# nabeelre/BTSbot

Measured on AMD Instinct MI355X. Metric: alerts/sec (63×63×3 triplet + 25 meta) train+infer, 1/2/4/8 MI355X, higher is better.
Workload: dtype bf16; 1 GPU; BASELINE.json configs[1]: ConvNeXt-pico multi-modal (mm_ConvNeXt) bf16 inference, batch=1024 synthetic triplets per GPU, inputs resident in HBM, logits+scores out; per_gpu_batch=1024, global_batch=1024, precision=bf16, weights=seeded random, layer-scale ~1, parallelism=1 independent replicas, batch-sharded, no collective, pipeline_depth=3

## Files before the change

btsbot_amd/csrc/device_math.h:

```cpp
#pragma once

struct h2x8 { f16x8 hi, lo; };
struct h2x4 { f16x4v hi, lo; };
__device__ __forceinline__ void split_f16(float v, _Float16& hi, _Float16& lo) {
  hi = (_Float16)v;
  lo = (_Float16)(v - (float)hi);
}
__device__ __forceinline__ h2x8 split8(const float (&v)[8]) {
  h2x8 o;
#pragma unroll
  for (int j = 0; j < 8; ++j) {
    _Float16 a, b;
    split_f16(v[j], a, b);
    o.hi[j] = a;
    o.lo[j] = b;
  }
  return o;
}
constexpr int AMAX_SUB = 16, AMAX_STRIDE = 32, AMAX_WORDS = AMAX_SUB * AMAX_STRIDE;
__device__ __forceinline__ int split_exp(const unsigned* amax) {
  if (amax == nullptr) return 0;
  unsigned m = 0;
#pragma unroll
  for (int i = 0; i < AMAX_SUB; ++i) m = max(m, amax[i * AMAX_STRIDE]);
// ... 38 lines not shown
template <> __device__ __forceinline__ float gelu_q<5>(float a) {
  float t = fmaf(a, -0.0004726569791655389f, 0.007079169600613161f);
  t = fmaf(a, t, -0.05181158088529847f);
  t = fmaf(a, t, -0.46001256950698816f);
  t = fmaf(a, t, -1.1507770495088248f);
  return fmaf(a, t, -1.000039487932206f);
}
__device__ __forceinline__ float relu_f(float x) {
  const int b = __float_as_int(x);
  return __int_as_float(b > 0 ? b : 0);
}
template <int DEG> __device__ __forceinline__ float gelu_poly(float x) {
  const float a = __builtin_fabsf(x);
  const float e = __builtin_amdgcn_exp2f(gelu_q<DEG>(a));
  return fmaf(-a, e, relu_f(x));
}
__device__ __forceinline__ void gelu_pk4(const float (&x)[8], f16x2v (&g)[4]) {
  const f16x2v c3 = {(_Float16)-0.024772998623334343f, (_Float16)-0.024772998623334343f};
  const f16x2v c2 = {(_Float16)-0.49926576060257244f, (_Float16)-0.49926576060257244f};
  const f16x2v c1 = {(_Float16)-1.1287482669759885f, (_Float16)-1.1287482669759885f};
  const f16x2v c0 = {(_Float16)-1.0036805164077327f, (_Float16)-1.0036805164077327f};
  const f16x2v z = {(_Float16)0.f, (_Float16)0.f};
  f16x2v xh[4], a[4], t[4];
  unsigned e[4];
#pragma unroll
  for (int i = 0; i < 4; ++i) xh[i] = __builtin_bit_cast(f16x2v, __builtin_amdgcn_cvt_pkrtz(x[2 * i], x[2 * i + 1]));
  __builtin_amdgcn_sched_barrier(0);
#pragma unroll
  for (int i = 0; i < 4; ++i) a[i] = __builtin_bit_cast(f16x2v, __builtin_bit_cast(unsigned, xh[i]) & 0x7fff7fffu);
  __builtin_amdgcn_sched_barrier(0);
#pragma unroll
  for (int i = 0; i < 4; ++i) t[i] = __builtin_elementwise_fma(a[i], c3, c2);
  __builtin_amdgcn_sched_barrier(0);
#pragma unroll
  for (int i = 0; i < 4; ++i) t[i] = __builtin_elementwise_fma(a[i], t[i], c1);
  __builtin_amdgcn_sched_barrier(0);
#pragma unroll
  for (int i = 0; i < 4; ++i) t[i] = __builtin_elementwise_fma(a[i], t[i], c0);
  __builtin_amdgcn_sched_barrier(0);
#pragma unroll
  for (int i = 0; i < 4; ++i) xh[i] = __builtin_elementwise_max(xh[i], z);
  __builtin_amdgcn_sched_barrier(0);
#pragma unroll
  for (int i = 0; i < 4; ++i) asm volatile("v_exp_f16_e32 %0, %1" : "=&v"(e[i]) : "v"(__builtin_bit_cast(unsigned, t[i])));
#pragma unroll
  for (int i = 0; i < 4; ++i)
    asm volatile("v_exp_f16_sdwa %0, %1 dst_sel:WORD_1 dst_unused:UNUSED_PRESERVE src0_sel:WORD_1"
                 : "+v"(e[i]) : "v"(__builtin_bit_cast(unsigned, t[i])));
  asm volatile("s_nop 0");
  __builtin_amdgcn_sched_barrier(0);
#pragma unroll
  for (int i = 0; i < 4; ++i) g[i] = __builtin_elementwise_fma(-a[i], __builtin_bit_cast(f16x2v, e[i]), xh[i]);
}
template <int DEG> __device__ __forceinline__ float gelu_dq(float a);
template <> __device__ __forceinline__ float gelu_dq<3>(float a) {
  float t = fmaf(a, 3.0f * -0.024772998623334343f, 2.0f * -0.49926576060257244f);
  return fmaf(a, t, -1.1287482669759885f);
}
template <> __device__ __forceinline__ float gelu_dq<5>(float a) {
  float t = fmaf(a, 5.0f * -0.0004726569791655389f, 4.0f * 0.007079169600613161f);
  t = fmaf(a, t, 3.0f * -0.05181158088529847f);
  t = fmaf(a, t, 2.0f * -0.46001256950698816f);
  return fmaf(a, t, -1.1507770495088248f);
}
template <int DEG> __device__ __forceinline__ float gelu_poly_grad(float x) {
  const float a = __builtin_fabsf(x);
  const float e = __builtin_amdgcn_exp2f(gelu_q<DEG>(a));
  const float d = e * fmaf(a * 0.6931471805599453f, gelu_dq<DEG>(a), 1.0f);
  return x > 0.0f ? 1.0f - d : d;
}
template <typename T> struct GeluDeg { static constexpr int value = 5; };
template <> struct GeluDeg<bf16_t> { static constexpr int value = 3; };
template <typename T> __device__ __forceinline__ float gelu_for(float x) { return gelu_poly<GeluDeg<T>::value>(x); }
template <> __device__ __forceinline__ float gelu_for<float>(float x) { return gelu_erf(x); }

__device__ __forceinline__ float gelu_grad(float x) {
  const float cdf = 0.5f * (1.0f + erff(x * 0.70710678118654752440f));
  const float pdf = 0.39894228040143267794f * __expf(-0.5f * x * x);
  return cdf + x * pdf;
}

__device__ __forceinline__ float silu_f(float x) { return x / (1.0f + __expf(-x)); }
__device__ __forceinline__ float silu_fast(float x) {
  return x * __builtin_amdgcn_rcpf(1.0f + __builtin_amdgcn_exp2f(-1.4426950408889634f * x));
}
template <typename T> __device__ __forceinline__ float silu_for(float x) { return silu_fast(x); }
template <> __device__ __forceinline__ float silu_for<float>(float x) { return silu_f(x); }

template <typename T> __device__ __forceinline__ float gelu_grad_for(float x) {
  return gelu_poly_grad<GeluDeg<T>::value>(x);
}
template <> __device__ __forceinline__ float gelu_grad_for<float>(float x) { return gelu_grad(x); }

template <typename T> __device__ __forceinline__ float to_f32(T x) { return (float)x; }

__device__ __forceinline__ float group16_sum(float v) {
#define BTS_DPP_ADD(ctrl)                                                                      \
  v += __builtin_bit_cast(float, __builtin_amdgcn_update_dpp(0, __builtin_bit_cast(int, v), ctrl, \
                                                             0xF, 0xF, true))
  BTS_DPP_ADD(0xB1);
  BTS_DPP_ADD(0x4E);
  BTS_DPP_ADD(0x141);
  BTS_DPP_ADD(0x140);
#undef BTS_DPP_ADD
  return v;
}
// ... 37 lines not shown
```

btsbot_amd/csrc/pack.hip:

```cpp
#include "ctx.h"
#include "head16.h"
#include "maxvit.h"
#include "stage3.h"

namespace {

template <typename T>
__global__ void cast_kernel(const float* __restrict__ s, T* __restrict__ d, int64_t n) {
  for (int64_t i = (int64_t)blockIdx.x * blockDim.x + threadIdx.x; i < n;
       i += (int64_t)gridDim.x * blockDim.x)
    d[i] = (T)s[i];
}

template <typename T>
__global__ void cast4_kernel(const float4* __restrict__ s, T* __restrict__ d, int64_t n4) {
  typedef __attribute__((ext_vector_type(4))) T t4;
  for (int64_t i = (int64_t)blockIdx.x * blockDim.x + threadIdx.x; i < n4;
       i += (int64_t)gridDim.x * blockDim.x) {
    const float4 v = s[i];
    *reinterpret_cast<t4*>(d + 4 * i) = t4{(T)v.x, (T)v.y, (T)v.z, (T)v.w};
  }
}

__global__ void transpose_kernel(const float* __restrict__ s, float* __restrict__ d, int R, int Cc) {
// ... 414 lines not shown
              [=](hipStream_t st) {
                return launch_pack_s2p(h->prec_down3(), h->mirror + d->w, nullptr, IMG(h, d->p_wp), ch, 4 * cin, 1, cin, nullptr, st);
              };
        job("down.p_w", &d->p_w, n * esz, FT, early && i == 1, PACK_DOWN, d->w, -1, ch, cin);
        job("down.p_wt", &d->p_wt, n * esz, if_tp, false, PACK_DOWN_T, d->w, -1, ch, cin);
        if (i == 3 && sc.stage2p)
          own("down.p_wp", &d->p_wp, 0, F, false, nullptr, [=](hipStream_t st) {
            return launch_pack_s2p(h->prec_down3(), h->mirror + d->w, nullptr, IMG(h, d->p_wp), ch, 4 * cin, 1, cin, nullptr, st);
          });
        if (i == 2 && sc.stage1)
          own("down.p_wp", &d->p_wp, n * esz, sc.s1_keep ? FT : F, false, nullptr, [=](hipStream_t st) {
            return launch_pack_frag32(h->prec_s01(), h->mirror + d->w, IMG(h, d->p_wp), ch, cin, st);
          });
        if (i == 1 && x2_s0) {
          own("down.p_x2_w", &d->p_x2_w, n * 2, F, false, nullptr, [=](hipStream_t st) {
            return launch_pack_down_split(h->mirror + d->w, IMG(h, d->p_x2_w), IMG(h, d->p_x2_wlo), ch, cin, st);
          });
          own("down.p_x2_wlo", &d->p_x2_wlo, n * 2, F, false, nullptr, nullptr);
        }
      }
      for (BlockPk& blk : h->blocks[i]) {
        BlockPk* b = &blk;
        const bool b_early = early && i == 0;
        job("p_dw", &b->p_dw, (size_t)49 * ch * 4, FT, b_early, PACK_TRANSPOSE_F32, b->dw_w, -1, ch, 49);
        job("p_fc1", &b->p_fc1, wb * esz, FT, b_early, PACK_CAST, b->fc1_w, -1, 4 * ch * ch, 1);
        job("p_fc2", &b->p_fc2, wb * esz, FT, false, PACK_CAST, b->fc2_w, -1, 4 * ch * ch, 1);
        const bool frag = (i == 2 && sc.stage2p) || (i == 3 && sc.stage3);
        if (i == 2 && sc.stage2p) {
          const unsigned t = sc.s2_keep ? IN_TRAIN : 0;
          job("p_w1p", &b->p_w1p, wb * esz, t, false, PACK_FRAG, b->fc1_w, -1, 4 * ch, ch).launch = [=](hipStream_t st) {
            return launch_pack_s2p(h->prec_tail(), h->mirror + b->fc1_w, nullptr, IMG(h, b->p_w1p), 4 * ch, ch, 0, 0,
                                   reinterpret_cast<float*>(IMG(h, b->p_scales)), st);
          };
          job("p_w2p", &b->p_w2p, wb * esz, t, false, PACK_FRAG, b->fc2_w, b->gamma, ch, 4 * ch).launch = [=](hipStream_t st) {
            return launch_pack_s2p(h->prec_tail(), h->mirror + b->fc2_w, h->mirror + b->gamma, IMG(h, b->p_w2p), ch, 4 * ch, 0, 0,
                                   reinterpret_cast<float*>(IMG(h, b->p_scales)) + 2, st);
          };
        }
        job("p_fc1t", &b->p_fc1t, wb * esz, if_tp, false, PACK_TRANSPOSE_CAST, b->fc1_w, -1, 4 * ch, ch);
        job("p_fc2t", &b->p_fc2t, wb * esz, if_tp, false, PACK_TRANSPOSE_CAST, b->fc2_w, b->gamma, ch, 4 * ch);
        if (!h->x2 && s2mlp_bwd_supported(prec, ch)) {
          const unsigned t = tp && sc.s2mlp ? FT : 0;
          ImageEntry& e1 = job("p_w1tp", &b->p_w1tp, wb * 2, t, false, PACK_TFRAG, b->fc1_w, -1, 4 * ch, ch);
          e1.reads = &b->p_fc1t;
          e1.launch = [=](hipStream_t st) { return launch_pack_frag16(IMG(h, b->p_fc1t), IMG(h, b->p_w1tp), ch, 4 * ch, st); };
          ImageEntry& e2 = job("p_w2tp", &b->p_w2tp, wb * 2, t, false, PACK_TFRAG, b->fc2_w, b->gamma, ch, 4 * ch);
          e2.reads = &b->p_fc2t;
          e2.launch = [=](hipStream_t st) { return launch_pack_frag16(IMG(h, b->p_fc2t), IMG(h, b->p_w2tp), 4 * ch, ch, st); };
        }
        own("p_fc2g", &b->p_fc2g, wb * esz, F | ((i == 0 && sc.s0_keep) || (i == 1 && sc.s1_keep) ? IN_TRAIN : 0), b_early, nullptr,
            [=](hipStream_t st) {
              return launch_rowscale_cast(h->cfg.precision, h->mirror + b->fc2_w, h->mirror + b->gamma, IMG(h, b->p_fc2g), ch, 4 * ch, st);
            });
        if (i == 0 && sc.stage0 && h->prec_s01() == BTSBOT_BF16)
          own("p_fc2g_h", &b->p_fc2g_h, wb * 2, F, false, nullptr, [=](hipStream_t st) {
            return launch_rowscale_cast(BTSBOT_F16, h->mirror + b->fc2_w, h->mirror + b->gamma, IMG(h, b->p_fc2g_h), ch, 4 * ch, st);
          });
        if (frag) {
          const bool s3 = i == 3;
          own("p_scales", &b->p_scales, 64, 0, false, nullptr, nullptr);
          own("p_w1p", &b->p_w1p, s3 ? wb * esz : 0, F, false, nullptr, [=](hipStream_t st) {
            float* sc = reinterpret_cast<float*>(IMG(h, b->p_scales));
            const float* w = h->mirror + b->fc1_w;
            return s3 ? launch_pack_s3(h->prec_tail(), w, nullptr, IMG(h, b->p_w1p), 4 * ch, ch, 1, sc, st)
                      : launch_pack_s2p(h->prec_tail(), w, nullptr, IMG(h, b->p_w1p), 4 * ch, ch, 0, 0, sc, st);
          });
          own("p_w2p", &b->p_w2p, s3 ? wb * esz : 0, F, false, nullptr, [=](hipStream_t st) {
            float* sc = reinterpret_cast<float*>(IMG(h, b->p_scales)) + 2;
            const float *w = h->mirror + b->fc2_w, *g = h->mirror + b->gamma;
            return s3 ? launch_pack_s3(h->prec_tail(), w, g, IMG(h, b->p_w2p), ch, 4 * ch, 0, sc, st)
                      : launch_pack_s2p(h->prec_tail(), w, g, IMG(h, b->p_w2p), ch, 4 * ch, 0, 0, sc, st);
          });
        }
        if (i == 1 && sc.stage1)
          own("p_s0par", &b->p_s0par, s1par_bytes(), F, false, &b->p_dw, [=](hipStream_t st) {
            const float* m = h->mirror;
            return launch_pack_s1par(h->prec_s01(), IMG_F32(h, b->p_dw), m + b->dw_b, m + b->ln_w, m + b->ln_b, IMG(h, b->p_s0par), st);
          });
        if (i == 0 && sc.stage0)
          own("p_s0par", &b->p_s0par, s0par_bytes(), F, false, &b->p_dw, [=](hipStream_t st) {
            const float* m = h->mirror;
            return launch_pack_s0par(h->prec_s01(), IMG_F32(h, b->p_dw), m + b->dw_b, m + b->ln_w, m + b->ln_b, m + b->fc1_b,
                                     m + b->fc2_b, m + b->gamma, IMG(h, b->p_s0par), st);
          });
        if (i == 1 && sc.s1_keep)
          own("p_s0par_t", &b->p_s0par_t, s1par_bytes(), if_tp, false, &b->p_dw, [=](hipStream_t st) {
            const float* m = h->mirror;
            return launch_pack_s1par(BTSBOT_F16, IMG_F32(h, b->p_dw), m + b->dw_b, m + b->ln_w, m + b->ln_b, IMG(h, b->p_s0par_t), st);
          });
        if (i == 0 && sc.s0_keep)
          own("p_s0par_t", &b->p_s0par_t, s0par_bytes(), if_tp, b_early, &b->p_dw, [=](hipStream_t st) {
            const float* m = h->mirror;
            return launch_pack_s0par(BTSBOT_F16, IMG_F32(h, b->p_dw), m + b->dw_b, m + b->ln_w, m + b->ln_b, m + b->fc1_b,
                                     m + b->fc2_b, m + b->gamma, IMG(h, b->p_s0par_t), st);
          });
        if (h->x2 && ((i == 0 && sc.stage0) || (i == 1 && sc.stage1))) {
          own("p_x2_w1", &b->p_x2_w1, wb * 2, F, false, nullptr, [=](hipStream_t st) {
            return launch_cast(BTSBOT_F16, h->mirror + b->fc1_w, IMG(h, b->p_x2_w1), (int64_t)4 * ch * ch, st);
          });
          own("p_x2_w2g", &b->p_x2_w2g, wb * 2, F, false, nullptr, [=](hipStream_t st) {
            return launch_rowscale_cast(BTSBOT_F16, h->mirror + b->fc2_w, h->mirror + b->gamma, IMG(h, b->p_x2_w2g), ch, 4 * ch, st);
          });
          own("p_x2_w1lo", &b->p_x2_w1lo, wb * 2, F, false, nullptr, [=](hipStream_t st) {
            return launch_rowscale_cast_lo(h->mirror + b->fc1_w, nullptr, IMG(h, b->p_x2_w1lo), 4 * ch, ch, st);
          });
          own("p_x2_w2glo", &b->p_x2_w2glo, wb * 2, F, false, nullptr, [=](hipStream_t st) {
            return launch_rowscale_cast_lo(h->mirror + b->fc2_w, h->mirror + b->gamma, IMG(h, b->p_x2_w2glo), ch, 4 * ch, st);
// ... 229 lines not shown
```

btsbot_amd/csrc/stage1b.hip:

```cpp
#include "stage0.h"
#include "stage_regs.h"
#include <type_traits>

namespace {

constexpr int C = 128, HW = 7, PA = 49, G = 2, NPX = G * PA, CT = 4, HID = 512, KS1 = 8;
constexpr int CN = 256, PO = 9;
constexpr int PITCH = 2 * C + 16;
static_assert(C == StageRegs<CT>::C && PITCH == StageRegs<CT>::PITCH, "ln_regs / regs_to_map derive both from CT");
constexpr int MAPB = NPX * PITCH;
constexpr int CHUNKB = 16384, HALFB = CHUNKB / 2, NCH = HID / 32, NSLOT = 3;
constexpr int PL_ROW = 136 * 8, PL_XQ = 8 * PL_ROW, PL_AL = 2 * PL_XQ, PLB = G * PL_AL;
constexpr int OFF_PL = 2 * CHUNKB;
constexpr int LNP = 4 * C + 16;
template <bool X2> struct S1L {
  static constexpr int PLANES = X2 ? 2 : 1;
  static constexpr int SLB = X2 ? 2 * HALFB : HALFB;
  static constexpr int OFF_W2X = OFF_PL + PLANES * PLB;
  static constexpr int OFF_B1 = OFF_W2X + (X2 ? 2 * SLB : 0);
  static constexpr int OFF_LNW = OFF_B1 + (HID + C) * 4;
  static constexpr int LDS_BYTES = OFF_LNW + 2 * C * 4;
  static_assert(4 * SLB <= PLANES * PLB, "W1 slots + W2 slot 0 inside the planar images");
  static_assert(NPX * LNP <= OFF_PL + PLB && NPX * LNP <= OFF_B1, "the fp32 image lies in ring slots 0, 1 + the planar image");
};
static_assert(MAPB <= 2 * CHUNKB && S1L<false>::LDS_BYTES <= 75264 && S1L<true>::LDS_BYTES <= 160 * 1024, "LDS layout");
constexpr int TW_R = 21, TW_BYTES = TW_R * C * 4 * 4 * 2;
constexpr int PARB = TW_BYTES + 3 * C * 4;
constexpr int PARB_X2 = 2 * TW_BYTES + 3 * C * 4;

#define SC_STAMP(i)                                                                \
  do {                                                                             \
    if (a.stamps != nullptr && blockIdx.x == 0 && threadIdx.x == 0) a.stamps[i] = clock64(); \
    if (a.wgt != nullptr && threadIdx.x == 0 && ((i) == 0 || (i) == 13))           \
      a.wgt[2 * blockIdx.x + ((i) == 13)] = wall_clock64();                        \
  } while (0)

template <typename T, int LOPLANE = 0, bool SAT = false>
__device__ __forceinline__ void regs_to_planar(const f32x16 (&x)[CT], unsigned char* pl, int p, int h) {
  const int al = p >= PA ? 1 : 0, pp = p - al * PA;
  const int y = pp / HW, xx = pp - y * HW;
  unsigned char* dst = pl + al * PL_AL + (xx >> 2) * PL_XQ + y * PL_ROW + (xx & 3) * 2 + h * 32;
#pragma unroll
  for (int ct = 0; ct < CT; ++ct)
#pragma unroll
    for (int r = 0; r < 16; ++r) {
      const T hi = (T)(SAT ? __builtin_amdgcn_fmed3f(x[ct][r], -65504.0f, 65504.0f) : x[ct][r]);
      *reinterpret_cast<T*>(dst + (ct * 32 + 8 * (r >> 2) + (r & 3)) * 8) = hi;
      if (LOPLANE > 0) *reinterpret_cast<T*>(dst + LOPLANE + (ct * 32 + 8 * (r >> 2) + (r & 3)) * 8) = (T)(x[ct][r] - (float)hi);
    }
}

template <typename T, bool X2, int WPS = 2, bool KEEP = false>
__global__ __launch_bounds__(256, WPS) void stage1b_kernel(Stage1Args a) {
  using frag = typename Mfma<T>::frag;
  using DT = typename std::conditional<KEEP, f16_t, T>::type;
  using frag4 = typename Mfma<DT>::frag4;
  extern __shared__ __attribute__((aligned(16))) unsigned char smem[];
  unsigned char* pl = smem + OFF_PL;
  unsigned char* stg = smem;
  using L = S1L<X2>;
  constexpr int SLB = L::SLB;
  constexpr int PLO = X2 ? PLB : 0;
  float* b1s = reinterpret_cast<float*>(smem + L::OFF_B1);
  float* b2s = b1s + HID;
  float* lnws = reinterpret_cast<float*>(smem + L::OFF_LNW);
  float* lnbs = lnws + C;
  auto w1slot = [&](int sl) { return pl + sl * SLB; };
  auto w2slot = [&](int sl) { return sl == 0 ? pl + 3 * SLB : (X2 ? smem + L::OFF_W2X : smem) + (sl - 1) * SLB; };

  const int tid = threadIdx.x, lane = tid & 63, wave = __builtin_amdgcn_readfirstlane(tid >> 6);
  const int lr = lane & 31, h = lane >> 5;
  const bool w1wave = wave < 2;
  const int a0 = blockIdx.x * G;
  const int nal = min(G, a.B - a0);
  const int p = wave * 32 + lr;
  const bool live = p < nal * PA;
  const bool inmap = p < NPX;
  const int pm = inmap ? p : 0;
  const int lnrow = pm * LNP + h * 32;
  SC_STAMP(0);
  auto zero_pads = [&]() {
#pragma unroll
    for (int pn = 0; pn < L::PLANES; ++pn) {
      unsigned char* pb = pl + pn * PLB;
      for (int i = tid; i < 4 * PL_ROW / 16; i += 256) {
        const int blk = i / (PL_ROW / 16), o = i - blk * (PL_ROW / 16);
        *reinterpret_cast<uint4*>(pb + (blk >> 1) * PL_AL + (blk & 1) * PL_XQ + 7 * PL_ROW + o * 16) = make_uint4(0u, 0u, 0u, 0u);
      }
      for (int i = tid; i < G * HW * C; i += 256) {
        const int al = i / (HW * C), r = (i / C) % HW, c = i % C;
        *reinterpret_cast<unsigned short*>(pb + al * PL_AL + PL_XQ + r * PL_ROW + c * 8 + 6) = 0;
      }
    }
  };
  zero_pads();
  const float* xsrc = a.x_in + ((size_t)a0 * PA + (live ? p : 0)) * C;
  float* xscr = a.scratch + ((size_t)a0 * PA + (live ? p : 0)) * C;
  auto load_x = [&](const float* src, f32x16 (&x)[CT]) {
#pragma unroll
    for (int ct = 0; ct < CT; ++ct)
#pragma unroll
      for (int qd = 0; qd < 4; ++qd) {
        const float4 v4 = *reinterpret_cast<const float4*>(src + ct * 32 + 8 * qd + 4 * h);
        x[ct][4 * qd + 0] = live ? v4.x : 0.f;
        x[ct][4 * qd + 1] = live ? v4.y : 0.f;
        x[ct][4 * qd + 2] = live ? v4.z : 0.f;
        x[ct][4 * qd + 3] = live ? v4.w : 0.f;
// ... 287 lines not shown
#define LS(i) do { __builtin_amdgcn_sched_barrier(0); if (ch == 6 || ch == 7) lts[i + 8 * (ch - 6)] = __builtin_amdgcn_s_memtime(); __builtin_amdgcn_sched_barrier(0); } while (0)
#else
#define LS(i)
#endif
      f32x16 hacc[2];
      frag a1[KS1];
      {
        wait_vm<(X2 ? 8 : 4) + 16>();
        asm volatile("s_waitcnt lgkmcnt(0)" ::: "memory");
        __builtin_amdgcn_s_barrier();
        bias_acc(0, hacc[0]);
        read_a1(0, a1);
#pragma unroll
        for (int ks = 0; ks < KS1; ++ks) {
          if (X2) {
            hacc[0] = Mfma<T>::m32(a1l[ks], xf[ks], hacc[0]);
            hacc[0] = Mfma<T>::m32(a1[ks], xfl[ks], hacc[0]);
          }
          hacc[0] = Mfma<T>::m32(a1[ks], xf[ks], hacc[0]);
        }
        __builtin_amdgcn_sched_barrier(0);
        wait_vm<0>();
        asm volatile("s_waitcnt lgkmcnt(0)" ::: "memory");
        __builtin_amdgcn_s_barrier();
        bias_acc(1, hacc[1]);
        read_a1(1, a1);
        __builtin_amdgcn_sched_barrier(0);
#pragma unroll
        for (int ct = 0; ct < CT; ++ct)
#pragma unroll
          for (int qd = 0; qd < 4; ++qd) {
            const f32x4 bv = lds4(b2s + ct * 32 + 8 * qd + 4 * h);
            const float4 v4 = xt[4 * ct + qd];
            x[ct][4 * qd + 0] = (live ? v4.x : 0.f) + bv[0];
            x[ct][4 * qd + 1] = (live ? v4.y : 0.f) + bv[1];
            x[ct][4 * qd + 2] = (live ? v4.z : 0.f) + bv[2];
            x[ct][4 * qd + 3] = (live ? v4.w : 0.f) + bv[3];
          }
#pragma unroll
        for (int ct = 0; ct < CT; ++ct) asm volatile("" : "+v"(x[ct]));
        __builtin_amdgcn_sched_barrier(0);
        if (w1wave) issue(3);
      }
      auto step = [&](auto last_c, int ch, f32x16& hc, f32x16& hn) {
        constexpr bool LAST = decltype(last_c)::value;
        LS(0);
        wait_vm<X2 ? 8 : 4>();
        LS(1);
        asm volatile("s_waitcnt lgkmcnt(0)" ::: "memory");
#ifndef S1_EXP_NOBAR
        __builtin_amdgcn_s_barrier();
#endif
        LS(2);
        frag a2[CT][2], a2l[X2 ? CT : 1][2];
        const unsigned char* w2s = w2slot(ch % NSLOT);
#pragma unroll
        for (int ct = 0; ct < CT; ++ct)
#pragma unroll
          for (int s2 = 0; s2 < 2; ++s2) {
            const int r = ct * 32 + lr;
            a2[ct][s2] = *reinterpret_cast<const frag*>(w2s + r * 64 + (((s2 * 2 + h) ^ swz4(r)) << 4));
            if (X2) a2l[ct][s2] = *reinterpret_cast<const frag*>(w2s + HALFB + r * 64 + (((s2 * 2 + h) ^ swz4(r)) << 4));
          }
        LS(3);
        const int kdma = ch + (w1wave ? 4 : 2);
        __builtin_amdgcn_sched_barrier(0);
        LS(4);
        float g[16];
#pragma unroll
        for (int r = 0; r < 8; ++r) {
          if (!LAST) {
            if (X2) {
              hn = Mfma<T>::m32(a1l[r], xf[r], hn);
              hn = Mfma<T>::m32(a1[r], xfl[r], hn);
            }
            hn = Mfma<T>::m32(a1[r], xf[r], hn);
          }
#ifdef S1_EXP_NOGELU
          g[r] = hc[r];
#else
          g[r] = gelu_for<T>(hc[r]);
#endif
#ifndef S1_EXP_NODMA
          if (X2) issue_piece(kdma, r);
          else if (r & 1) issue_piece(kdma, r >> 1);
#endif
          __builtin_amdgcn_sched_barrier(0);
        }
        LS(5);
        if (!LAST) read_a1(ch + 2, a1);
        frag hf, hfl;
#pragma unroll
        for (int r = 0; r < 8; ++r) {
          hf[r] = (T)g[r];
          if (X2) hfl[r] = (T)(g[r] - (float)hf[r]);
        }
#pragma unroll
        for (int ct = 0; ct < CT; ++ct) {
          if (X2) {
            x[ct] = Mfma<T>::m32(a2l[ct][0], hf, x[ct]);
            x[ct] = Mfma<T>::m32(a2[ct][0], hfl, x[ct]);
          }
          x[ct] = Mfma<T>::m32(a2[ct][0], hf, x[ct]);
#ifdef S1_EXP_NOGELU
          g[8 + 2 * ct] = hc[8 + 2 * ct];
          g[9 + 2 * ct] = hc[9 + 2 * ct];
#else
          g[8 + 2 * ct] = gelu_for<T>(hc[8 + 2 * ct]);
          g[9 + 2 * ct] = gelu_for<T>(hc[9 + 2 * ct]);
#endif
          __builtin_amdgcn_sched_barrier(0);
        }
        if (!LAST) bias_acc(ch + 2, hc);
#pragma unroll
        for (int r = 0; r < 8; ++r) {
          hf[r] = (T)g[8 + r];
          if (X2) hfl[r] = (T)(g[8 + r] - (float)hf[r]);
        }
        LS(6);
#pragma unroll
        for (int ct = 0; ct < CT; ++ct) {
          if (X2) {
            x[ct] = Mfma<T>::m32(a2l[ct][1], hf, x[ct]);
            x[ct] = Mfma<T>::m32(a2[ct][1], hfl, x[ct]);
          }
          x[ct] = Mfma<T>::m32(a2[ct][1], hf, x[ct]);
        }
        LS(7);
      };
#ifndef S1_EXP_NOLOOP
#pragma unroll 1
      for (int ch = 0; ch < NCH - 2; ch += 2) {
        step(std::false_type{}, ch, hacc[0], hacc[1]);
        step(std::false_type{}, ch + 1, hacc[1], hacc[0]);
      }
      step(std::false_type{}, NCH - 2, hacc[0], hacc[1]);
      step(std::true_type{}, NCH - 1, hacc[1], hacc[0]);
#endif
      asm volatile("s_waitcnt lgkmcnt(0)" ::: "memory");
#ifdef S1_LOOPSTAMP
      if (a.wgt != nullptr && blockIdx.x == 0 && tid == 0 && j == 0)
        for (int i = 0; i < 16; ++i) a.wgt[4096 + i] = lts[i];
#endif
      wait_vm<0>();
      if (j == 0) {
        __syncthreads();
        zero_pads();
        if (inmap) regs_to_planar<DT, PLO, KEEP && !std::is_same<T, f16_t>::value>(x, pl, p, h);
        if (live) {
#pragma unroll
          for (int ct = 0; ct < CT; ++ct)
#pragma unroll
            for (int qd = 0; qd < 4; ++qd)
              *reinterpret_cast<float4*>(xscr + ct * 32 + 8 * qd + 4 * h) =
                  make_float4(x[ct][4 * qd], x[ct][4 * qd + 1], x[ct][4 * qd + 2], x[ct][4 * qd + 3]);
        }
      }
    }
    SC_STAMP(6 + 5 * j);
  }
  if (a.tap_stage != nullptr && live) {
    float* tp = a.tap_stage + ((size_t)a0 * PA + p) * C;
#pragma unroll
    for (int ct = 0; ct < CT; ++ct)
#pragma unroll
      for (int qd = 0; qd < 4; ++qd)
        *reinterpret_cast<float4*>(tp + ct * 32 + 8 * qd + 4 * h) =
            make_float4(x[ct][4 * qd], x[ct][4 * qd + 1], x[ct][4 * qd + 2], x[ct][4 * qd + 3]);
  }

  {
    __syncthreads();
    {
      f32x16 xn[CT];
      ln_regs(x, a.ds_lnw, a.ds_lnb, h, xn);
      if (inmap) regs_to_map<T, X2 ? MAPB : 0>(xn, stg, p, h);
    }
    static_assert(2 * MAPB <= L::OFF_B1, "two [pixel][channel] images in front of the bias words");
    constexpr int KSD = 4 * C / 16, RING = X2 ? 8 : 16, NSTEP = 2 * KSD;
// ... 68 lines not shown
          *reinterpret_cast<float4*>(dst + 8 * qd) =
              make_float4(acc[4 * qd], acc[4 * qd + 1], acc[4 * qd + 2], acc[4 * qd + 3]);
      }
    }
    SC_STAMP(13);
  }
}

template <typename T, bool X2>
__global__ void pack_s1par_kernel(const float* __restrict__ taps, const float* __restrict__ dw_b,
                                  const float* __restrict__ ln_w, const float* __restrict__ ln_b,
                                  unsigned char* __restrict__ out) {
  const int idx = blockIdx.x * blockDim.x + threadIdx.x;
  constexpr int NTW = TW_R * C * 16;
  if (idx < NTW) {
    const int k = idx & 3, i = (idx >> 2) & 3, c = (idx >> 4) & (C - 1), r = idx / (16 * C);
    const int ky = r / 3, rb = r % 3 - 1, kx = 4 * rb + k - i + 3;
    const float w = (kx >= 0 && kx < 7) ? taps[(ky * 7 + kx) * C + c] : 0.f;
    const T wh = (T)w;
    reinterpret_cast<T*>(out)[idx] = wh;
    if (X2) reinterpret_cast<T*>(out)[NTW + idx] = (T)(w - (float)wh);
    return;
  }
  const int f = idx - NTW;
  if (f >= 3 * C) return;
  float v;
  if (f < C) v = dw_b[f];
  else if (f < 2 * C) v = ln_w[f - C];
  else v = ln_b[f - 2 * C];
  reinterpret_cast<float*>(out + (X2 ? 2 : 1) * TW_BYTES)[f] = v;
}

template <typename T, bool X2 = false>
__global__ void pack_frag32_kernel(const float* __restrict__ w, T* __restrict__ out, int rows, int cin) {
  const long i = (long)blockIdx.x * blockDim.x + threadIdx.x;
  const int K = 4 * cin;
  if (i >= (long)rows * K) return;
  const int j = (int)(i & 7), l = (int)((i >> 3) & 63);
  const long fs = i >> 9;
  const int ksteps = K / 16;
  const int sk = (int)(fs % ksteps), tile = (int)(fs / ksteps);
  const int row = 32 * tile + (l & 31), k = 16 * sk + 8 * (l >> 5) + j;
  const int q = k / cin, c = k - q * cin;
  const float v = w[((long)row * cin + c) * 4 + q];
  const T vh = (T)v;
  if (X2) {
    out[fs * 1024 + l * 8 + j] = vh;
    out[fs * 1024 + 512 + l * 8 + j] = (T)(v - (float)vh);
  } else {
    out[i] = vh;
  }
}

template <typename T, bool X2 = false, int WPS = 2, bool KEEP = false> int launch_stage1b_t(const Stage1Args& a, hipStream_t st) {
  auto kern = stage1b_kernel<T, X2, WPS, KEEP>;
  static DevOnce attr_set;
  static const int pad = switch_on(SW_S1_ONE_WG) && !X2 ? 90 * 1024 - S1L<X2>::LDS_BYTES : 0;
  const int LDS_BYTES = S1L<X2>::LDS_BYTES + pad;
  if (attr_set.need()) {
    HIP_TRY(hipFuncSetAttribute(reinterpret_cast<const void*>(kern),
                                hipFuncAttributeMaxDynamicSharedMemorySize, (int)LDS_BYTES));
    attr_set.done();
  }
  hipLaunchKernelGGL(kern, dim3((a.B + G - 1) / G), dim3(256), LDS_BYTES, st, a);
  LAUNCH_CHECK();
  return BTSBOT_OK;
}

}

#ifdef STAGE1B_X2_TU
int launch_stage1b_x2(const Stage1Args& a, hipStream_t st) {
  if (a.blk[0].w1_lo == nullptr || a.blk[0].w2g_lo == nullptr || a.blk[1].w1_lo == nullptr || a.blk[1].w2g_lo == nullptr) {
    btsbot_set_error("stage1b: the split mode needs the filters' remainder images (w1_lo, w2g_lo)");
    return BTSBOT_ERR_INVALID_ARG;
  }
  return launch_stage1b_t<f16_t, true, 1>(a, st);
}
int launch_pack_s1par_x2(const float* taps, const float* dw_b, const float* ln_w, const float* ln_b, void* out,
                         hipStream_t st) {
  const dim3 grid((TW_R * C * 16 + 3 * C + 255) / 256), blk(256);
  hipLaunchKernelGGL((pack_s1par_kernel<f16_t, true>), grid, blk, 0, st, taps, dw_b, ln_w, ln_b,
                     reinterpret_cast<unsigned char*>(out));
  LAUNCH_CHECK();
  return BTSBOT_OK;
}
int launch_pack_frag32_x2(const float* src, void* dst, int cout, int cin, hipStream_t st) {
  const long total = (long)cout * 4 * cin;
  hipLaunchKernelGGL((pack_frag32_kernel<f16_t, true>), dim3((unsigned)((total + 255) / 256)), dim3(256), 0, st, src,
                     reinterpret_cast<f16_t*>(dst), cout, cin);
  LAUNCH_CHECK();
  return BTSBOT_OK;
}
#else
int launch_stage1b_x2(const Stage1Args& a, hipStream_t st);
int launch_pack_s1par_x2(const float* taps, const float* dw_b, const float* ln_w, const float* ln_b, void* out,
                         hipStream_t st);
int launch_pack_frag32_x2(const float* src, void* dst, int cout, int cin, hipStream_t st);

size_t s1par_bytes() { return PARB_X2; }

int launch_pack_s1par(int prec, const float* taps, const float* dw_b, const float* ln_w,
                      const float* ln_b, void* out, hipStream_t st) {
  unsigned char* o = reinterpret_cast<unsigned char*>(out);
  const dim3 grid((TW_R * C * 16 + 3 * C + 255) / 256), blk(256);
  if (prec == BTSBOT_BF16)
    hipLaunchKernelGGL((pack_s1par_kernel<bf16_t, false>), grid, blk, 0, st, taps, dw_b, ln_w, ln_b, o);
  else if (prec == BTSBOT_F16)
    hipLaunchKernelGGL((pack_s1par_kernel<f16_t, false>), grid, blk, 0, st, taps, dw_b, ln_w, ln_b, o);
  else if (prec == BTSBOT_F16X2)
    return launch_pack_s1par_x2(taps, dw_b, ln_w, ln_b, out, st);
  else {
    btsbot_set_error("pack_s1par: precision %d is not a 16-bit mode", prec);
    return BTSBOT_ERR_INVALID_ARG;
  }
  LAUNCH_CHECK();
  return BTSBOT_OK;
}

int launch_pack_frag32(int prec, const float* src, void* dst, int cout, int cin, hipStream_t st) {
  const long total = (long)cout * 4 * cin;
  const dim3 grid((unsigned)((total + 255) / 256)), blk(256);
  if (prec == BTSBOT_BF16)
    hipLaunchKernelGGL(pack_frag32_kernel<bf16_t>, grid, blk, 0, st, src, reinterpret_cast<bf16_t*>(dst), cout, cin);
  else if (prec == BTSBOT_F16)
    hipLaunchKernelGGL(pack_frag32_kernel<f16_t>, grid, blk, 0, st, src, reinterpret_cast<f16_t*>(dst), cout, cin);
  else if (prec == BTSBOT_F16X2)
    return launch_pack_frag32_x2(src, dst, cout, cin, st);
  else {
    btsbot_set_error("pack_frag32: precision %d is not a 16-bit mode", prec);
    return BTSBOT_ERR_INVALID_ARG;
  }
  LAUNCH_CHECK();
  return BTSBOT_OK;
}

bool stage1_supported(int prec, int c1, int c2) {
  return (prec == BTSBOT_BF16 || prec == BTSBOT_F16 || prec == BTSBOT_F16X2) && c1 == 128 && c2 == 256;
}

int launch_stage1b(int prec, const Stage1Args& a, hipStream_t st) {
  if (a.B <= 0) return BTSBOT_OK;
  if (a.keep_xn[0] != nullptr) {
    if ((a.keep_d[0] == nullptr) != (a.keep_d[1] == nullptr) || a.keep_xn[1] == nullptr || a.keep_patches == nullptr ||
        a.tap_stage == nullptr || a.scratch == nullptr) {
      btsbot_set_error("stage1b: the training forward needs every kept buffer");
      return BTSBOT_ERR_INVALID_ARG;
    }
    if (prec == BTSBOT_BF16) return launch_stage1b_t<bf16_t, false, 2, true>(a, st);
    if (prec == BTSBOT_F16) return launch_stage1b_t<f16_t, false, 2, true>(a, st);
    btsbot_set_error("stage1b: the training forward runs in the bf16 / f16 modes, not %d", prec);
    return BTSBOT_ERR_INVALID_ARG;
  }
  if (prec == BTSBOT_BF16) return launch_stage1b_t<bf16_t>(a, st);
  if (prec == BTSBOT_F16) return launch_stage1b_t<f16_t>(a, st);
  if (prec == BTSBOT_F16X2) return launch_stage1b_x2(a, st);
  btsbot_set_error("stage1b: unsupported precision %d", prec);
  return BTSBOT_ERR_INVALID_ARG;
}
#endif
```

btsbot_amd/csrc/stage_args.hip:

```cpp
#include <string.h>

#include "ctx.h"
#include "stage0.h"
#include "stage2p.h"
#include "stage3.h"

namespace {

int s01_blk(const btsbot_ctx* h, const BlockPk& b, bool keep, bool hid16, Stage0Blk* out) {
  const float* m = h->mirror;
  const bool x2 = h->x2 && !keep;
  Stage0Blk& k = *out;
  k.dw_w = IMG_F32(h, b.p_dw);
  k.dw_b = m + b.dw_b;
  k.ln_w = m + b.ln_w;
  k.ln_b = m + b.ln_b;
  k.b1 = m + b.fc1_b;
  k.b2 = m + b.fc2_b;
  k.gamma = m + b.gamma;
  k.w1 = x2 ? IMG(h, b.p_x2_w1) : IMG(h, b.p_fc1);
  k.par = keep ? IMG(h, b.p_s0par_t) : IMG(h, b.p_s0par);
  k.w2g = x2 ? IMG(h, b.p_x2_w2g) : hid16 ? IMG(h, b.p_fc2g_h) : IMG(h, b.p_fc2g);
  k.w1_lo = x2 ? IMG(h, b.p_x2_w1lo) : nullptr;
  k.w2g_lo = x2 ? IMG(h, b.p_x2_w2glo) : nullptr;
  return BTSBOT_OK;
}

}

int stage0_args(const btsbot_ctx* h, bool keep, Stage0Args* out) {
  const float* m = h->mirror;
  const bool x2 = h->x2 && !keep;
  const DownPk& d = h->down[1];
  Stage0Args& a = *out;
  memset(&a, 0, sizeof(a));
  a.stem_w = x2 ? IMG(h, h->p_x2_stem) : IMG(h, h->p_stem16);
  a.stem_w_lo = x2 ? IMG(h, h->p_x2_stemlo) : nullptr;
  a.stem_b = m + h->stem_b;
  a.stem_lnw = m + h->stem_lnw;
  a.stem_lnb = m + h->stem_lnb;
  for (int j = 0; j < 2; ++j) {
    const int s = s01_blk(h, h->blocks[0][j], keep, !keep && h->prec_s01() == BTSBOT_BF16, &a.blk[j]);
    if (s != BTSBOT_OK) return s;
  }
  a.ds_lnw = m + d.ln_w;
  a.ds_lnb = m + d.ln_b;
  a.ds_w = x2 ? IMG(h, d.p_x2_w) : IMG(h, d.p_w);
  a.ds_w_lo = x2 ? IMG(h, d.p_x2_wlo) : nullptr;
  a.ds_b = m + d.b;
  return BTSBOT_OK;
}

int stage1_args(const btsbot_ctx* h, bool keep, Stage1Args* out) {
  const float* m = h->mirror;
  const DownPk& d = h->down[2];
  Stage1Args& a = *out;
  memset(&a, 0, sizeof(a));
  for (int j = 0; j < 2; ++j) {
    const int s = s01_blk(h, h->blocks[1][j], keep, false, &a.blk[j]);
    if (s != BTSBOT_OK) return s;
  }
  a.ds_lnw = m + d.ln_w;
  a.ds_lnb = m + d.ln_b;
  a.ds_w = IMG(h, d.p_wp);
  a.ds_b = m + d.b;
  return BTSBOT_OK;
}

int stage2p_args(const btsbot_ctx* h, bool keep, Stage2pArgs* out) {
  const float* m = h->mirror;
  const DownPk& d = h->down[3];
  Stage2pArgs& a = *out;
  memset(&a, 0, sizeof(a));
  a.depth = (int)h->blocks[2].size();
  for (int j = 0; j < a.depth; ++j) {
    const BlockPk& b = h->blocks[2][j];
    Stage2pBlk& k = a.blk[j];
    k.dw_w = IMG_F32(h, b.p_dw);
    k.dw_b = m + b.dw_b;
    k.ln_w = m + b.ln_w;
    k.ln_b = m + b.ln_b;
    k.b1 = m + b.fc1_b;
    k.b2 = m + b.fc2_b;
    k.gamma = m + b.gamma;
    k.w1p = IMG(h, b.p_w1p);
    k.w2p = IMG(h, b.p_w2p);
    k.scales = h->fp8 && !keep ? IMG_F32(h, b.p_scales) : nullptr;
  }
  a.ds_lnw = m + d.ln_w;
  a.ds_lnb = m + d.ln_b;
  a.ds_wp = IMG(h, d.p_wp);
  a.ds_b = m + d.b;
  a.cw = h->cfg.dims[2];
  a.alerts_hint = h->sched.s2p_alerts;
  return BTSBOT_OK;
}

int stage3_args(const btsbot_ctx* h, Stage3Args* out) {
  const float* m = h->mirror;
  const int ch = h->cfg.dims[3];
  Stage3Args& a = *out;
  memset(&a, 0, sizeof(a));
  a.depth = (int)h->blocks[3].size();
  for (int j = 0; j < a.depth; ++j) {
    const BlockPk& b = h->blocks[3][j];
    Stage3Blk& k = a.blk[j];
    k.dw_c = IMG_F32(h, b.p_dw) + 24 * ch;
    k.dw_b = m + b.dw_b;
    k.ln_w = m + b.ln_w;
    k.ln_b = m + b.ln_b;
    k.w1p = IMG(h, b.p_w1p);
    k.b1 = m + b.fc1_b;
// ... 8 lines not shown
```

Measured before the change: 4.036 million alerts/s.

## Use packed f16 GELU and f16 fc2 weights in stage1 bf16 inference

In bf16 inference, the stage1 block now computes GELU on packed f16 pairs through a staged helper. The packed GELU steps are interleaved with the fc1 and fc2 MFMAs and the weight DMA issues, so VALU work hides under matrix ops. The fc2 hidden operand uses f16 MFMA with a new f16 row-scaled fc2 weight copy, packed for stage1 as well as stage0. This removes the per-element fp32 GELU and conversion work, at the cost of a degree-3 f16 GELU approximation with lower precision.

```diff
diff --git a/btsbot_amd/csrc/device_math.h b/btsbot_amd/csrc/device_math.h
--- a/btsbot_amd/csrc/device_math.h
+++ b/btsbot_amd/csrc/device_math.h
@@ -114,6 +114,49 @@
 #pragma unroll
   for (int i = 0; i < 4; ++i) g[i] = __builtin_elementwise_fma(-a[i], __builtin_bit_cast(f16x2v, e[i]), xh[i]);
 }
+struct GeluPk4 {
+  f16x2v xh[4], a[4], t[4];
+  unsigned e[4];
+  static __device__ __forceinline__ void here(const f16x2v (&v)[4]) {
+    asm volatile("" ::"v"(v[0]), "v"(v[1]), "v"(v[2]), "v"(v[3]));
+    __builtin_amdgcn_sched_barrier(0);
+  }
+  __device__ __forceinline__ void begin(const float (&x)[8]) {
+#pragma unroll
+    for (int i = 0; i < 4; ++i) xh[i] = __builtin_bit_cast(f16x2v, __builtin_amdgcn_cvt_pkrtz(x[2 * i], x[2 * i + 1]));
+    here(xh);
+  }
+  template <int S> __device__ __forceinline__ void stage() {
+    static_assert(S >= 1 && S <= 7, "begin(), stage<1>() .. stage<7>(), finish()");
+    const f16x2v c3 = {(_Float16)-0.024772998623334343f, (_Float16)-0.024772998623334343f};
+    const f16x2v c2 = {(_Float16)-0.49926576060257244f, (_Float16)-0.49926576060257244f};
+    const f16x2v c1 = {(_Float16)-1.1287482669759885f, (_Float16)-1.1287482669759885f};
+    const f16x2v c0 = {(_Float16)-1.0036805164077327f, (_Float16)-1.0036805164077327f};
+    const f16x2v z = {(_Float16)0.f, (_Float16)0.f};
+#pragma unroll
+    for (int i = 0; i < 4; ++i) {
+      if (S == 1) a[i] = __builtin_bit_cast(f16x2v, __builtin_bit_cast(unsigned, xh[i]) & 0x7fff7fffu);
+      if (S == 2) t[i] = __builtin_elementwise_fma(a[i], c3, c2);
+      if (S == 3) t[i] = __builtin_elementwise_fma(a[i], t[i], c1);
+      if (S == 4) t[i] = __builtin_elementwise_fma(a[i], t[i], c0);
+      if (S == 5) xh[i] = __builtin_elementwise_max(xh[i], z);
+      if (S == 6) asm volatile("v_exp_f16_e32 %0, %1" : "=&v"(e[i]) : "v"(__builtin_bit_cast(unsigned, t[i])));
+      if (S == 7)
+        asm volatile("v_exp_f16_sdwa %0, %1 dst_sel:WORD_1 dst_unused:UNUSED_PRESERVE src0_sel:WORD_1"
+                     : "+v"(e[i]) : "v"(__builtin_bit_cast(unsigned, t[i])));
+    }
+    if (S == 7) asm volatile("s_nop 0");
+    if (S == 1) here(a);
+    else if (S <= 4) here(t);
+    else if (S == 5) here(xh);
+    else __builtin_amdgcn_sched_barrier(0);
+  }
+  __device__ __forceinline__ void finish(f16x2v (&g)[4]) {
+#pragma unroll
+    for (int i = 0; i < 4; ++i) g[i] = __builtin_elementwise_fma(-a[i], __builtin_bit_cast(f16x2v, e[i]), xh[i]);
+    here(g);
+  }
+};
 template <int DEG> __device__ __forceinline__ float gelu_dq(float a);
 template <> __device__ __forceinline__ float gelu_dq<3>(float a) {
   float t = fmaf(a, 3.0f * -0.024772998623334343f, 2.0f * -0.49926576060257244f);
diff --git a/btsbot_amd/csrc/pack.hip b/btsbot_amd/csrc/pack.hip
--- a/btsbot_amd/csrc/pack.hip
+++ b/btsbot_amd/csrc/pack.hip
@@ -490,7 +490,7 @@
             [=](hipStream_t st) {
               return launch_rowscale_cast(h->cfg.precision, h->mirror + b->fc2_w, h->mirror + b->gamma, IMG(h, b->p_fc2g), ch, 4 * ch, st);
             });
-        if (i == 0 && sc.stage0 && h->prec_s01() == BTSBOT_BF16)
+        if (((i == 0 && sc.stage0) || (i == 1 && sc.stage1)) && h->prec_s01() == BTSBOT_BF16)
           own("p_fc2g_h", &b->p_fc2g_h, wb * 2, F, false, nullptr, [=](hipStream_t st) {
             return launch_rowscale_cast(BTSBOT_F16, h->mirror + b->fc2_w, h->mirror + b->gamma, IMG(h, b->p_fc2g_h), ch, 4 * ch, st);
           });
diff --git a/btsbot_amd/csrc/stage1b.hip b/btsbot_amd/csrc/stage1b.hip
--- a/btsbot_amd/csrc/stage1b.hip
+++ b/btsbot_amd/csrc/stage1b.hip
@@ -50,9 +50,12 @@
     }
 }
 
-template <typename T, bool X2, int WPS = 2, bool KEEP = false>
+template <typename T, bool X2, int WPS = 2, bool KEEP = false, typename HT = T>
 __global__ __launch_bounds__(256, WPS) void stage1b_kernel(Stage1Args a) {
   using frag = typename Mfma<T>::frag;
+  using hfrag = typename Mfma<HT>::frag;
+  constexpr bool PKG = !std::is_same<HT, T>::value;
+  static_assert(!PKG || (std::is_same<HT, f16_t>::value && !X2 && !KEEP), "a hidden type of its own: f16, inference, one operand");
   using DT = typename std::conditional<KEEP, f16_t, T>::type;
   using frag4 = typename Mfma<DT>::frag4;
   extern __shared__ __attribute__((aligned(16))) unsigned char smem[];
@@ -446,79 +449,155 @@
         __builtin_amdgcn_s_barrier();
 #endif
         LS(2);
-        frag a2[CT][2], a2l[X2 ? CT : 1][2];
+        hfrag a2[CT][2], a2l[X2 ? CT : 1][2];
         const unsigned char* w2s = w2slot(ch % NSLOT);
 #pragma unroll
         for (int ct = 0; ct < CT; ++ct)
 #pragma unroll
           for (int s2 = 0; s2 < 2; ++s2) {
             const int r = ct * 32 + lr;
-            a2[ct][s2] = *reinterpret_cast<const frag*>(w2s + r * 64 + (((s2 * 2 + h) ^ swz4(r)) << 4));
-            if (X2) a2l[ct][s2] = *reinterpret_cast<const frag*>(w2s + HALFB + r * 64 + (((s2 * 2 + h) ^ swz4(r)) << 4));
+            a2[ct][s2] = *reinterpret_cast<const hfrag*>(w2s + r * 64 + (((s2 * 2 + h) ^ swz4(r)) << 4));
+            if (X2) a2l[ct][s2] = *reinterpret_cast<const hfrag*>(w2s + HALFB + r * 64 + (((s2 * 2 + h) ^ swz4(r)) << 4));
           }
         LS(3);
         const int kdma = ch + (w1wave ? 4 : 2);
         __builtin_amdgcn_sched_barrier(0);
         LS(4);
-        float g[16];
-#pragma unroll
-        for (int r = 0; r < 8; ++r) {
-          if (!LAST) {
+        if constexpr (PKG) {
+          auto pk_frag = [](const f16x2v (&g2)[4]) {
+            return __builtin_shufflevector(__builtin_shufflevector(g2[0], g2[1], 0, 1, 2, 3),
+                                           __builtin_shufflevector(g2[2], g2[3], 0, 1, 2, 3), 0, 1, 2, 3, 4, 5, 6, 7);
+          };
+          const int sl = kdma % NSLOT;
+          const int o1 = OFF_PL + sl * SLB, o2 = sl == 0 ? OFF_PL + 3 * SLB : (sl - 1) * SLB;
+          unsigned dma_dst = (unsigned)(size_t)(lptr_t)(smem + (w1wave ? o1 : o2) + (wave & 1) * 4096);
+          unsigned dma_src = (unsigned)((kdma + rot) & (NCH - 1)) * (unsigned)wstep0;
+          asm volatile("" : "+s"(dma_dst), "+s"(dma_src));
+          GeluPk4 gp;
+          float hx[8];
+#pragma unroll
+          for (int r = 0; r < 8; ++r) hx[r] = hc[r];
+          auto fc1_gelu = [&](auto rc) {
+            constexpr int r = decltype(rc)::value;
+            if (!LAST) hn = Mfma<T>::m32(a1[r], xf[r], hn);
+            if constexpr (r == 0) gp.begin(hx);
+#ifndef S1_EXP_NOGELU
+            else gp.template stage<r>();
+#endif
+#ifndef S1_EXP_NODMA
+            if (r & 1)
+              __builtin_amdgcn_global_load_lds((gptr_t)(wsrc[r >> 1] + dma_src), (lptr_t)(size_t)(dma_dst + (r >> 1) * 1024), 16, 0, 0);
+#endif
+            __builtin_amdgcn_sched_barrier(0);
+          };
+          fc1_gelu(std::integral_constant<int, 0>{});
+          fc1_gelu(std::integral_constant<int, 1>{});
+          fc1_gelu(std::integral_constant<int, 2>{});
+          fc1_gelu(std::integral_constant<int, 3>{});
+          fc1_gelu(std::integral_constant<int, 4>{});
+          fc1_gelu(std::integral_constant<int, 5>{});
+          fc1_gelu(std::integral_constant<int, 6>{});
+          fc1_gelu(std::integral_constant<int, 7>{});
+          LS(5);
+          if (!LAST) read_a1(ch + 2, a1);
+          f16x2v g2[4];
+#ifdef S1_EXP_NOGELU
+#pragma unroll
+          for (int i = 0; i < 4; ++i) g2[i] = gp.xh[i];
+#else
+          gp.finish(g2);
+#endif
+          hfrag hf = pk_frag(g2);
+#pragma unroll
+          for (int r = 0; r < 8; ++r) hx[r] = hc[8 + r];
+          x[0] = Mfma<HT>::m32(a2[0][0], hf, x[0]);
+          gp.begin(hx);
+#ifndef S1_EXP_NOGELU
+          gp.template stage<1>();
+          gp.template stage<2>();
+          x[1] = Mfma<HT>::m32(a2[1][0], hf, x[1]);
+          gp.template stage<3>();
+          gp.template stage<4>();
+          gp.template stage<5>();
+          x[2] = Mfma<HT>::m32(a2[2][0], hf, x[2]);
+          gp.template stage<6>();
+          x[3] = Mfma<HT>::m32(a2[3][0], hf, x[3]);
+          gp.template stage<7>();
+          gp.finish(g2);
+#else
+          x[1] = Mfma<HT>::m32(a2[1][0], hf, x[1]);
+          x[2] = Mfma<HT>::m32(a2[2][0], hf, x[2]);
+          x[3] = Mfma<HT>::m32(a2[3][0], hf, x[3]);
+#pragma unroll
+          for (int i = 0; i < 4; ++i) g2[i] = gp.xh[i];
+          __builtin_amdgcn_sched_barrier(0);
+#endif
+          if (!LAST) bias_acc(ch + 2, hc);
+          hf = pk_frag(g2);
+          LS(6);
+#pragma unroll
+          for (int ct = 0; ct < CT; ++ct) x[ct] = Mfma<HT>::m32(a2[ct][1], hf, x[ct]);
+        } else {
+          float g[16];
+#pragma unroll
+          for (int r = 0; r < 8; ++r) {
+            if (!LAST) {
+              if (X2) {
+                hn = Mfma<T>::m32(a1l[r], xf[r], hn);
+                hn = Mfma<T>::m32(a1[r], xfl[r], hn);
+              }
+              hn = Mfma<T>::m32(a1[r], xf[r], hn);
+            }
+#ifdef S1_EXP_NOGELU
+            g[r] = hc[r];
+#else
+            g[r] = gelu_for<T>(hc[r]);
+#endif
+#ifndef S1_EXP_NODMA
+            if (X2) issue_piece(kdma, r);
+            else if (r & 1) issue_piece(kdma, r >> 1);
+#endif
+            __builtin_amdgcn_sched_barrier(0);
+          }
+          LS(5);
+          if (!LAST) read_a1(ch + 2, a1);
+          frag hf, hfl;
+#pragma unroll
+          for (int r = 0; r < 8; ++r) {
+            hf[r] = (T)g[r];
+            if (X2) hfl[r] = (T)(g[r] - (float)hf[r]);
+          }
+#pragma unroll
+          for (int ct = 0; ct < CT; ++ct) {
             if (X2) {
-              hn = Mfma<T>::m32(a1l[r], xf[r], hn);
-              hn = Mfma<T>::m32(a1[r], xfl[r], hn);
+              x[ct] = Mfma<T>::m32(a2l[ct][0], hf, x[ct]);
+              x[ct] = Mfma<T>::m32(a2[ct][0], hfl, x[ct]);
             }
-            hn = Mfma<T>::m32(a1[r], xf[r], hn);
-          }
+            x[ct] = Mfma<T>::m32(a2[ct][0], hf, x[ct]);
 #ifdef S1_EXP_NOGELU
-          g[r] = hc[r];
+            g[8 + 2 * ct] = hc[8 + 2 * ct];
+            g[9 + 2 * ct] = hc[9 + 2 * ct];
 #else
-          g[r] = gelu_for<T>(hc[r]);
-#endif
-#ifndef S1_EXP_NODMA
-          if (X2) issue_piece(kdma, r);
-          else if (r & 1) issue_piece(kdma, r >> 1);
-#endif
-          __builtin_amdgcn_sched_barrier(0);
-        }
-        LS(5);
-        if (!LAST) read_a1(ch + 2, a1);
-        frag hf, hfl;
-#pragma unroll
-        for (int r = 0; r < 8; ++r) {
-          hf[r] = (T)g[r];
-          if (X2) hfl[r] = (T)(g[r] - (float)hf[r]);
-        }
-#pragma unroll
-        for (int ct = 0; ct < CT; ++ct) {
-          if (X2) {
-            x[ct] = Mfma<T>::m32(a2l[ct][0], hf, x[ct]);
-            x[ct] = Mfma<T>::m32(a2[ct][0], hfl, x[ct]);
-          }
-          x[ct] = Mfma<T>::m32(a2[ct][0], hf, x[ct]);
-#ifdef S1_EXP_NOGELU
-          g[8 + 2 * ct] = hc[8 + 2 * ct];
-          g[9 + 2 * ct] = hc[9 + 2 * ct];
-#else
-          g[8 + 2 * ct] = gelu_for<T>(hc[8 + 2 * ct]);
-          g[9 + 2 * ct] = gelu_for<T>(hc[9 + 2 * ct]);
-#endif
-          __builtin_amdgcn_sched_barrier(0);
-        }
-        if (!LAST) bias_acc(ch + 2, hc);
-#pragma unroll
-        for (int r = 0; r < 8; ++r) {
-          hf[r] = (T)g[8 + r];
-          if (X2) hfl[r] = (T)(g[8 + r] - (float)hf[r]);
-        }
-        LS(6);
-#pragma unroll
-        for (int ct = 0; ct < CT; ++ct) {
-          if (X2) {
-            x[ct] = Mfma<T>::m32(a2l[ct][1], hf, x[ct]);
-            x[ct] = Mfma<T>::m32(a2[ct][1], hfl, x[ct]);
-          }
-          x[ct] = Mfma<T>::m32(a2[ct][1], hf, x[ct]);
+            g[8 + 2 * ct] = gelu_for<T>(hc[8 + 2 * ct]);
+            g[9 + 2 * ct] = gelu_for<T>(hc[9 + 2 * ct]);
+#endif
+            __builtin_amdgcn_sched_barrier(0);
+          }
+          if (!LAST) bias_acc(ch + 2, hc);
+#pragma unroll
+          for (int r = 0; r < 8; ++r) {
+            hf[r] = (T)g[8 + r];
+            if (X2) hfl[r] = (T)(g[8 + r] - (float)hf[r]);
+          }
+          LS(6);
+#pragma unroll
+          for (int ct = 0; ct < CT; ++ct) {
+            if (X2) {
+              x[ct] = Mfma<T>::m32(a2l[ct][1], hf, x[ct]);
+              x[ct] = Mfma<T>::m32(a2[ct][1], hfl, x[ct]);
+            }
+            x[ct] = Mfma<T>::m32(a2[ct][1], hf, x[ct]);
+          }
         }
         LS(7);
       };
@@ -693,8 +772,9 @@
   }
 }
 
-template <typename T, bool X2 = false, int WPS = 2, bool KEEP = false> int launch_stage1b_t(const Stage1Args& a, hipStream_t st) {
-  auto kern = stage1b_kernel<T, X2, WPS, KEEP>;
+template <typename T, bool X2 = false, int WPS = 2, bool KEEP = false, typename HT = T>
+int launch_stage1b_t(const Stage1Args& a, hipStream_t st) {
+  auto kern = stage1b_kernel<T, X2, WPS, KEEP, HT>;
   static DevOnce attr_set;
   static const int pad = switch_on(SW_S1_ONE_WG) && !X2 ? 90 * 1024 - S1L<X2>::LDS_BYTES : 0;
   const int LDS_BYTES = S1L<X2>::LDS_BYTES + pad;
@@ -793,7 +873,7 @@
     btsbot_set_error("stage1b: the training forward runs in the bf16 / f16 modes, not %d", prec);
     return BTSBOT_ERR_INVALID_ARG;
   }
-  if (prec == BTSBOT_BF16) return launch_stage1b_t<bf16_t>(a, st);
+  if (prec == BTSBOT_BF16) return launch_stage1b_t<bf16_t, false, 2, false, f16_t>(a, st);
   if (prec == BTSBOT_F16) return launch_stage1b_t<f16_t>(a, st);
   if (prec == BTSBOT_F16X2) return launch_stage1b_x2(a, st);
   btsbot_set_error("stage1b: unsupported precision %d", prec);
diff --git a/btsbot_amd/csrc/stage_args.hip b/btsbot_amd/csrc/stage_args.hip
--- a/btsbot_amd/csrc/stage_args.hip
+++ b/btsbot_amd/csrc/stage_args.hip
@@ -57,7 +57,7 @@
   Stage1Args& a = *out;
   memset(&a, 0, sizeof(a));
   for (int j = 0; j < 2; ++j) {
-    const int s = s01_blk(h, h->blocks[1][j], keep, false, &a.blk[j]);
+    const int s = s01_blk(h, h->blocks[1][j], keep, !keep && h->prec_s01() == BTSBOT_BF16, &a.blk[j]);
     if (s != BTSBOT_OK) return s;
   }
   a.ds_lnw = m + d.ln_w;
```

After: 4.075 million alerts/s, median of 6. Within noise of the previous version (+1.0%).
